# mbjd/binaural-audio-synthesis

Measured on AMD Instinct MI355X. Metric: stereo samples/sec, 256 concurrent moving sources @44.1kHz mixed to one stereo pair (x real-time in x_realtime), higher is better.
Workload: dtype f32

## Files before the change

binaural-audio-synthesis_amd/csrc/bas_fused_split.hip:

```cpp
#include "bas_fused.h"

#ifndef FZ_NT_LOADS
#define FZ_NT_LOADS 1
#endif

#ifndef FS_PSPLIT
#define FS_PSPLIT 1
#endif
#ifndef FS_STAGER_PRIO
#define FS_STAGER_PRIO 3
#endif
#ifndef FS_FILTER_PRIO
#define FS_FILTER_PRIO 0
#endif

#ifdef BAS_STAMPS
__device__ unsigned long long bas_fs_stamps[1024 * 8 * 8];
#define FS_NOW() __builtin_amdgcn_s_memrealtime()
#else
#define FS_NOW() 0ull
#endif

#if FZ_ASM
template <int UNITLEN, int NSUB = 1, int PSPLIT = 0>
__global__ __launch_bounds__(512, 1) void bas_render_fs_kernel(
    FzArgs A, const float *__restrict__ x,
    float *__restrict__ slab,
    const float *__restrict__ packed,
    const unsigned *__restrict__ plans,
    float *__restrict__ y, unsigned int *__restrict__ peak_bits) {
    constexpr int NW = 4;
    constexpr int THREADS = 64 * NW;
    constexpr int TILE = 2048 * NW;
    constexpr int ROWS = TILE / 32 + HD_HALO;
    constexpr int XR = ROWS + 1;
    constexpr int NX = (ROWS * 8 + THREADS - 1) / THREADS;
    constexpr int XFLOATS = 8 * XR * 4;
    constexpr int MAXEV = BAS_FS_MAXEV;
    constexpr int PL4 = 2 * BAS_PLANS_WORDS / 4;
    constexpr int NPV = (MAXEV * PL4 + 63) / 64;
    static_assert(XR == 261, "bas_fir_asm.inc holds the row step for this x-image stride");
    extern __shared__ f32x4 lds4[];
    const int buf4 = (XFLOATS + ((A.nslots * HD_SLOT + 3) & ~3)) / 4;
    f32x4 *pl_base = lds4 + 2 * buf4;
    f32x4 *bnd = pl_base + NW * (MAXEV * PL4);
    volatile unsigned *flags = reinterpret_cast<volatile unsigned *>(bnd + NW * 64);

    const int tid0 = threadIdx.x;
    const int lane0 = tid0 & 63;
    const int wv8 = __builtin_amdgcn_readfirstlane(tid0 >> 6);
    const bool stager = wv8 >= NW;
    const int wv = wv8 & (NW - 1);

    const long unit0 = (long)blockIdx.x * A.units_per_wg;
    long unit1 = unit0 + A.units_per_wg;
    if (unit1 > A.units_total) unit1 = A.units_total;
    const int nseg = (A.Lp + RT_SEG - 1) / RT_SEG;
    const long n_pass = (unit1 - unit0) * nseg;
    if (!A.direct && peak_bits && blockIdx.x == 0 && tid0 == 0) *peak_bits = 0u;
    if (n_pass <= 0) {
        if (A.direct && A.tail_mode) bas_tail<2 * THREADS>(fz_tail(A, y, peak_bits), 0.f);
        return;
    }
    unsigned wmax_bits = 0u;
    if (tid0 < NW) flags[tid0] = 0u;
    __syncthreads();

    const long first_tile = unit0 / A.n_src;
    long tile = first_tile;
    int s = (int)(unit0 - first_tile * A.n_src);
    int sg = 0;
    struct Geo {
        int seg0, Lseg, halo, nrows, c0, mo0;
        long xbase;
    };
    auto make_geo = [&](long t, int g) {
        Geo G;
        G.seg0 = g * RT_SEG;
        G.Lseg = A.Lp - G.seg0 < RT_SEG ? A.Lp - G.seg0 : RT_SEG;
        G.halo = (G.Lseg + 31) >> 5;
        G.xbase = t * TILE - G.seg0 - 32L * G.halo;
        G.nrows = TILE / 32 + G.halo;
        long cf = G.xbase / A.K;
        if (cf * A.K > G.xbase) --cf;
        G.c0 = (int)cf;
        G.mo0 = (int)(G.xbase - cf * A.K);
        return G;
    };
    Geo G = make_geo(tile, sg);
    auto advance = [&]() {
        int n_sg = sg + 1;
        long n_tile = tile;
        if (n_sg == nseg) {
            n_sg = 0;
            if (++s == A.n_src) {
                s = 0;
                ++n_tile;
            }
        }
        if (n_tile != tile || n_sg != sg) G = make_geo(n_tile, n_sg);
        tile = n_tile;
        sg = n_sg;
    };
#ifdef BAS_STAMPS
    unsigned long long st_work = 0, st_wait = 0, st_clk = 0;
    const unsigned long long st_begin = FS_NOW(), st_begin_clk = __builtin_amdgcn_s_memtime();
#endif

    if (!stager) {
        if (FS_FILTER_PRIO) __builtin_amdgcn_s_setprio(FS_FILTER_PRIO);
        static_assert(!PSPLIT || (NSUB == 1 && UNITLEN != 0), "the P split exists for the unit blocks of subchunks >= 32");
        f32x32 accA, accB, accP;
        f32x2 accB16 = f32x2{0.f, 0.f};
        f32x16 accPA, accPB, accPP;
        f32x2 accPB8 = f32x2{0.f, 0.f};
#pragma unroll
        for (int i = 0; i < 32; ++i) accA[i] = accB[i] = accP[i] = 0.f;
#pragma unroll
        for (int i = 0; i < 16; ++i) accPA[i] = accPB[i] = accPP[i] = 0.f;
        float *slab_wg = slab + (long)blockIdx.x * A.parts_per_wg * 2 * TILE;
        auto flush = [&](long t) {
            f32x2 acc[32];
            if constexpr (PSPLIT) {
#pragma unroll
                for (int r = 0; r < 8; ++r) {
                    const f32x2 a = f32x2{accPA[2 * r], accPA[2 * r + 1]}, b0 = f32x2{accPB[2 * r], accPB[2 * r + 1]};
                    const f32x2 b1 = r < 7 ? f32x2{accPB[2 * r + 2], accPB[2 * r + 3]} : accPB8;
                    const f32x2 pp = f32x2{accPP[2 * r], accPP[2 * r + 1]};
                    const f32x2 pe = a + b0, po = (pp - a) - b1;
                    accP[4 * r] = pe.x; accP[4 * r + 1] = pe.y;
                    accP[4 * r + 2] = po.x; accP[4 * r + 3] = po.y;
                }
            }
#pragma unroll
            for (int p = 0; p < 16; ++p) {
                const f32x2 a = f32x2{accA[2 * p], accA[2 * p + 1]}, b0 = f32x2{accB[2 * p], accB[2 * p + 1]};
                const f32x2 b1 = p < 15 ? f32x2{accB[2 * p + 2], accB[2 * p + 3]} : accB16;
                const f32x2 pp = f32x2{accP[2 * p], accP[2 * p + 1]};
                acc[2 * p] = a + b0;
                acc[2 * p + 1] = (pp - a) - b1;
            }
#pragma unroll
            for (int i = 0; i < 32; ++i) accA[i] = accB[i] = accP[i] = 0.f;
            accB16 = f32x2{0.f, 0.f};
            if constexpr (PSPLIT) {
#pragma unroll
                for (int i = 0; i < 16; ++i) accPA[i] = accPB[i] = accPP[i] = 0.f;
                accPB8 = f32x2{0.f, 0.f};
            }
            if (A.direct) {
                const long n0 = t * TILE + 2048 * wv + 32 * lane0;
                const float lmax = fz_store_row_direct(acc, y, A.T_out, n0, A.accumulate);
                if (A.tail_mode) {
                    const unsigned b = fz_wave_max_bits(lmax);
                    wmax_bits = b > wmax_bits ? b : wmax_bits;
                } else if (peak_bits) {
                    bas_wave_peak_max(lmax, peak_bits);
                }
                return;
            }
            float *dst = slab_wg + (t - first_tile) * 2 * TILE + 2048 * wv + 32 * lane0;
            f32x4 *l4 = reinterpret_cast<f32x4 *>(dst);
            f32x4 *r4 = reinterpret_cast<f32x4 *>(dst + TILE);
#pragma unroll
            for (int i = 0; i < 8; ++i) {
                l4[i] = f32x4{acc[4 * i].x, acc[4 * i + 1].x, acc[4 * i + 2].x, acc[4 * i + 3].x};
                r4[i] = f32x4{acc[4 * i].y, acc[4 * i + 1].y, acc[4 * i + 2].y, acc[4 * i + 3].y};
            }
        };
        long open_tile = -1;
        long addr_tile = -1;
        int addr_buf = 0;
        unsigned tapv[5] = {0u, 0u, 0u, 0u, 0u}, xrow4 = 0u;
        float alv[5] = {0.f, 0.f, 0.f, 0.f, 0.f}, blv[5] = {0.f, 0.f, 0.f, 0.f, 0.f};
        const unsigned buf_bytes = 16u * (unsigned)buf4;
        for (long pid = 0; pid < n_pass; ++pid) {
            int tid = tid0;
            asm volatile("" : "+v"(tid));
            const int lane = tid & 63;
#ifdef BAS_STAMPS
            const unsigned long long t0 = FS_NOW();
#endif
            if (tile != open_tile) {
                if (open_tile >= 0) flush(open_tile);
                open_tile = tile;
            }
            auto weight = [&](int m) {
                if (A.s_pow2) return (float)(m & ~(A.S - 1)) * A.invK;
                int q = (int)((float)m * A.invS);
                const int r = m - q * A.S;
                if (r < 0) q -= 1;
                if (r >= A.S) q += 1;
                return (float)(q * A.S) * A.invK;
            };
            if constexpr (UNITLEN != 0) {
                const int cur_buf = (int)(pid & 1);
                const long akey = tile * nseg + sg;
                if (akey == addr_tile && cur_buf != addr_buf) {
                    const unsigned delta = cur_buf ? buf_bytes : 0u - buf_bytes;
#pragma unroll
                    for (int r = 0; r < 5; ++r) tapv[r] += delta;
                    xrow4 += delta;
                    addr_buf = cur_buf;
                }
                if (akey != addr_tile) {
                    addr_tile = akey;
                    addr_buf = cur_buf;
                    const unsigned bufb = (unsigned)reinterpret_cast<uintptr_t>(lds4 + cur_buf * buf4);
                    const int row_out = 64 * wv + lane + G.halo;
                    const int pos = G.mo0 + 32 * row_out;
                    int sl = (int)((float)pos * A.invK);
                    int m_in = pos - sl * A.K;
                    if (m_in < 0) { m_in += A.K; sl -= 1; }
                    if (m_in >= A.K) { m_in -= A.K; sl += 1; }
                    xrow4 = bufb + 16u * (unsigned)(row_out - 4);
                    unsigned tap = bufb + 4u * (unsigned)(XFLOATS + sl * HD_SLOT - 32 * 4);
#pragma unroll
                    for (int r = 0; r < 5; ++r) {
                        alv[r] = weight(m_in);
                        if constexpr (NSUB == 2) blv[r] = weight(m_in + 16);
                        tapv[r] = tap;
                        m_in -= 32;
                        const bool wrap = m_in < 0;
                        m_in += wrap ? A.K : 0;
                        tap += 32u * 16u - (wrap ? 4u * (unsigned)HD_SLOT : 0u);
                    }
                }
            }
#ifdef BAS_STAMPS
            const unsigned long long t1 = FS_NOW();
#endif
            __syncthreads();
#ifdef BAS_STAMPS
            const unsigned long long t2 = FS_NOW();
#endif
            const f32x4 *xs4 = lds4 + (pid & 1) * buf4;
            const float *hd = reinterpret_cast<const float *>(xs4) + XFLOATS;
            const int Lseg = G.Lseg, halo = G.halo;
#ifdef BAS_STAMPS
            const unsigned long long c0 = __builtin_amdgcn_s_memtime();
#endif
            if constexpr (UNITLEN != 0) {
                if constexpr (PSPLIT)
                    ffa_unitp_asm<XR, UNITLEN>(accA, accB, accPA, accPB, accPB8, accPP, accB16, xrow4, tapv, alv);
                else if constexpr (NSUB == 4)
                    ffa_unit4_asm<XR, UNITLEN>(accA, accB, accB16, accP, xrow4, tapv, alv, (float)A.S * A.invK);
                else if constexpr (NSUB == 2)
                    ffa_unit2_asm<XR, UNITLEN>(accA, accB, accB16, accP, xrow4, tapv, alv, blv);
                else
                    ffa_unit_asm<XR, UNITLEN>(accA, accB, accB16, accP, xrow4, tapv, alv);
                (void)hd; (void)Lseg; (void)halo;
            } else {
                const int row_out = 64 * wv + lane + halo;
                const int pos = G.mo0 + 32 * row_out;
                int sl = (int)((float)pos * A.invK);
                int m_in = pos - sl * A.K;
                if (m_in < 0) { m_in += A.K; sl -= 1; }
                if (m_in >= A.K) { m_in -= A.K; sl += 1; }
                const f32x4 *xrow = xs4 + row_out;
#pragma unroll 1
                for (int rp = 0; rp <= halo; ++rp) {
                    float al;
                    if (A.s_pow2) {
                        al = (float)(m_in & ~(A.S - 1)) * A.invK;
                    } else {
                        int q = (int)((float)m_in * A.invS);
                        const int r = m_in - q * A.S;
                        if (r < 0) q -= 1;
                        if (r >= A.S) q += 1;
                        al = (float)(q * A.S) * A.invK;
                    }
                    const int oct_lo = 4 - 4 * rp > 0 ? 4 - 4 * rp : 0;
                    int oct_hi = (Lseg + 32 - 32 * rp) >> 3;
                    oct_hi = oct_hi > 8 ? 8 : oct_hi;
                    const unsigned mk = ((1u << oct_hi) - 1u) & ~((1u << oct_lo) - 1u);
                    ffa_row_step_asm<XR>(accA, accB, accB16, accP, (unsigned)reinterpret_cast<uintptr_t>(xrow),
                                         (unsigned)reinterpret_cast<uintptr_t>(hd + sl * HD_SLOT + (32 * rp - 32) * 4), al, mk);
                    xrow -= 1;
                    m_in -= 32;
                    if (m_in < 0) {
                        m_in += A.K;
                        sl -= 1;
                    }
                }
            }
#ifdef BAS_STAMPS
            st_clk += __builtin_amdgcn_s_memtime() - c0;
            st_work += (t1 - t0) + (FS_NOW() - t2);
            st_wait += t2 - t1;
#endif
            advance();
        }
        flush(open_tile);
    } else {
        __builtin_amdgcn_s_setprio(FS_STAGER_PRIO);
        const __amdgpu_buffer_rsrc_t tab =
            __builtin_amdgcn_make_buffer_rsrc(const_cast<float *>(packed), 0, (int)A.packed_bytes, 0x00020000);
        const unsigned L4 = 4u * (unsigned)A.L;
        const int n_ir = A.nslots + 1, base = n_ir / NW, rem = n_ir - base * NW;
        const int slot_a = rfl(wv * base + (wv < rem ? wv : rem));
        const int slot_b = rfl(slot_a + base + (wv < rem ? 1 : 0));
        const int n_ev = slot_a < slot_b ? slot_b - slot_a : 0;
        const bool need_next = n_ev > 0 && slot_b <= A.nslots;
        f32x4 *plw = pl_base + wv * (MAXEV * PL4);
        const int tid = tid0 - THREADS;
        const int lane = tid & 63;
        const int half = lane >> 5;
        const int tq = 4 * (lane & 31) + (lane < 32 ? 2 : 0);
        const unsigned v16 = 16u * (unsigned)tid, l16 = 16u * (unsigned)lane;
        const bool all_live = A.L == A.Lp;
        for (long pid = 0; pid < n_pass; ++pid) {
#ifdef BAS_STAMPS
            const unsigned long long t0 = FS_NOW();
#endif
#ifndef FS_NO_STAGE
            f32x4 *xs4 = lds4 + (pid & 1) * buf4;
            float *hd = reinterpret_cast<float *>(xs4) + XFLOATS;
            const int seg0 = G.seg0, Lseg = G.Lseg, nrows = G.nrows;
            const long xbase = G.xbase;
            f32x4 pv[NPV], xv[NX];
            {
                const f32x4 *pl_src = reinterpret_cast<const f32x4 *>(plans) + (long)s * (A.n_chunks + 1) * PL4;
                const int c_first = rfl(G.c0 + slot_a);
                if (c_first >= 0 && c_first + n_ev - 1 <= A.n_chunks) {
                    const __amdgpu_buffer_rsrc_t pr = __builtin_amdgcn_make_buffer_rsrc(
                        const_cast<f32x4 *>(pl_src + (long)c_first * PL4), 0, n_ev * PL4 * 16, 0x00020000);
#pragma unroll
                    for (int r = 0; r < NPV; ++r)
                        pv[r] = __builtin_bit_cast(f32x4, __builtin_amdgcn_raw_buffer_load_b128(pr, (int)l16, 1024 * r, FZ_NT_LOADS ? 2 : 0));
                } else {
#pragma unroll
                    for (int r = 0; r < NPV; ++r) {
                        int p = lane + 64 * r;
                        p = p < n_ev * PL4 ? p : 0;
                        const int i = (p * 3641) >> 16;
                        const int c = clampi(c_first + i, 0, A.n_chunks);
#if FZ_NT_LOADS
                        pv[r] = __builtin_nontemporal_load(pl_src + (long)c * PL4 + (p - i * PL4));
#else
                        pv[r] = pl_src[(long)c * PL4 + (p - i * PL4)];
#endif
                    }
                }
            }
            const long lo_l = -xbase, hi_l = A.T_in - xbase;
            const int x_lo = lo_l < -(1 << 30) ? -(1 << 30) : (lo_l > (1 << 30) ? (1 << 30) : (int)lo_l);
            const int x_hi = hi_l < -(1 << 30) ? -(1 << 30) : (hi_l > (1 << 30) ? (1 << 30) : (int)hi_l);
            const bool x_inside = x_lo <= 0 && x_hi >= 4 * NX * THREADS;
            {
                const float *xwin = x + (long)s * A.x_stride + xbase;
                if (x_inside) {
                    const __amdgpu_buffer_rsrc_t xr = __builtin_amdgcn_make_buffer_rsrc(const_cast<float *>(xwin), 0,
                                                                                        16 * NX * THREADS, 0x00020000);
#pragma unroll
                    for (int j = 0; j < NX; ++j)
                        xv[j] = __builtin_bit_cast(f32x4, __builtin_amdgcn_raw_buffer_load_b128(xr, (int)v16, 16 * THREADS * j, FZ_NT_LOADS ? 2 : 0));
                } else {
                    asm volatile("" ::: "memory");
#pragma unroll
                    for (int j = 0; j < NX; ++j) {
                        int i = 4 * (tid + j * THREADS);
                        i = i < x_lo ? x_lo : i;
                        i = i > x_hi - 4 ? x_hi - 4 : i;
#if FZ_NT_LOADS
                        xv[j] = __builtin_nontemporal_load(reinterpret_cast<const f32x4 *>(xwin + i));
#else
                        xv[j] = *reinterpret_cast<const f32x4 *>(xwin + i);
#endif
                    }
                }
            }
            const unsigned pass_id = (unsigned)pid + 1u;
#pragma unroll
            for (int r = 0; r < NPV; ++r)
                if (lane + 64 * r < n_ev * PL4) plw[lane + 64 * r] = pv[r];
            {
                f32x4 *xcol = xs4 + (tid & 7) * XR + (tid >> 3);
                if (!x_inside) {
                    asm volatile("" ::: "memory");
#pragma unroll
                    for (int j = 0; j < NX; ++j) {
                        const int e = 4 * (tid + j * THREADS);
                        if (!(e >= x_lo && e < x_hi)) xv[j] = f32x4{0.f, 0.f, 0.f, 0.f};
                    }
                }
#pragma unroll
                for (int j = 0; j < NX; ++j) {
                    if ((j + 1) * THREADS <= (TILE / 32 + 1) * 8 || tid + j * THREADS < nrows * 8) xcol[32 * j] = xv[j];
                }
            }
            __builtin_amdgcn_wave_barrier();

            {
                const int m = seg0 + 4 * (lane & 31);
                const int m_c = m < A.L ? m : A.L - 1;
                const unsigned m4 = 4u * (unsigned)m_c;
                const f32x4 live = f32x4{m < A.L ? 1.f : 0.f, m + 1 < A.L ? 1.f : 0.f, m + 2 < A.L ? 1.f : 0.f,
                                         m + 3 < A.L ? 1.f : 0.f};
                const f32x4 *pl = plw + half * (BAS_PLANS_WORDS / 4);
                f32x4 *dst = reinterpret_cast<f32x4 *>(hd) + slot_a * (HD_SLOT / 4) + tq;
                FzHalf ha, hb;
                f32x2 pa = f32x2{0.f, 0.f}, pb = pa;
                const f32x4 *pl_last = pl + (n_ev > 0 ? n_ev - 1 : 0) * PL4;
                if (n_ev > 0) fz_issue<0>(tab, pl, m4, L4, ha);
                for (int i = 0; i < n_ev; ++i) {
                    const f32x4 *pl_next = pl + PL4 < pl_last ? pl + PL4 : pl_last;
                    fz_issue<1>(tab, pl, m4, L4, hb);
                    f32x4 h = fz_finish<0>(pl, ha, f32x4{0.f, 0.f, 0.f, 0.f});
                    fz_issue<0>(tab, pl_next, m4, L4, ha);
                    h = fz_finish<1>(pl, hb, h);
                    if (!all_live) h *= live;
                    if (i == 0 && wv > 0) {
                        bnd[wv * 64 + lane] = h;
                        __builtin_amdgcn_fence(__ATOMIC_RELEASE, "workgroup");
                        if (lane == 0 && !fz_inject(A)) flags[wv] = pass_id;
                    }
                    f32x2 ca, cb;
                    fz_pair_ears(h, ca, cb);
                    if (i > 0) {
                        const f32x2 da = ca - pa, db = cb - pb;
                        if (tq < Lseg) {
                            dst[0] = f32x4{pa.x, pa.y, da.x, da.y};
                            dst[1] = f32x4{pb.x, pb.y, db.x, db.y};
                        }
                        dst += HD_SLOT / 4;
                    }
                    pa = ca;
                    pb = cb;
                    pl = pl_next;
                }
                if (need_next) {
                    const bool got = fz_wait_handover(flags + wv + 1, pass_id, A);
                    __builtin_amdgcn_fence(__ATOMIC_ACQUIRE, "workgroup");
                    f32x4 nx = bnd[(wv + 1) * 64 + lane];
                    if (!got) nx = f32x4{__builtin_nanf(""), __builtin_nanf(""), __builtin_nanf(""), __builtin_nanf("")};
                    f32x2 ca, cb;
                    fz_pair_ears(nx, ca, cb);
                    const f32x2 da = ca - pa, db = cb - pb;
                    if (tq < Lseg) {
                        dst[0] = f32x4{pa.x, pa.y, da.x, da.y};
                        dst[1] = f32x4{pb.x, pb.y, db.x, db.y};
                    }
                }
            }
#endif
#ifdef BAS_STAMPS
            asm volatile("s_waitcnt vmcnt(0) lgkmcnt(0)" ::: "memory");
            const unsigned long long t1 = FS_NOW();
#endif
            __syncthreads();
#ifdef BAS_STAMPS
            st_work += t1 - t0;
            st_wait += FS_NOW() - t1;
#endif
            advance();
        }
    }
    if (A.direct && A.tail_mode) bas_tail<2 * THREADS>(fz_tail(A, y, peak_bits), __uint_as_float(wmax_bits));
#ifdef BAS_STAMPS
    if (lane0 == 0 && blockIdx.x < 1024) {
        unsigned long long *d = bas_fs_stamps + (blockIdx.x * 8 + wv8) * 8;
        d[0] = st_work;
        d[1] = st_wait;
        d[2] = st_clk;
        d[3] = __builtin_amdgcn_s_memtime() - st_begin_clk;
        d[6] = FS_NOW() - st_begin;
        d[7] = (unsigned long long)n_pass;
    }
#endif
}

#ifdef BAS_STAMPS
extern "C" int bas_debug_read_fs_stamps(unsigned long long *host, size_t count) {
    return (int)hipMemcpyFromSymbol(host, HIP_SYMBOL(bas_fs_stamps), count * sizeof(unsigned long long));
}
#endif

#endif

int bas_fs_unit_len(int Lp) {
    return FS_UNIT_BLOCK && (Lp == 104 || (Lp > 0 && Lp % 128 == 0)) ? (Lp == 104 ? 104 : 128) : 0;
}

size_t bas_fs_lds_bytes(int nslots) {
    const int rows = 8192 / 32 + HD_HALO;
    return (size_t)(2 * (8 * (rows + 1) * 4 + ((nslots * HD_SLOT + 3) & ~3)) + 4 * BAS_FS_MAXEV * 2 * BAS_PLANS_WORDS + 4 * 64 * 4 + 4) *
           sizeof(float);
}

hipError_t bas_fs_launch(const FzArgs &A, const float *x, float *slab, const float *packed, const unsigned *plans, float *y,
                         unsigned int *peak_bits, int n_wg, size_t lds_bytes, hipStream_t st, hipEvent_t eb, hipEvent_t ee) {
#if FZ_ASM
    typedef void (*fs_fn)(FzArgs, const float *, float *, const float *, const unsigned *, float *, unsigned int *);
    const int ul = bas_fs_unit_len(A.Lp);
#if FS_PSPLIT
    fs_fn fn = ul == 128 ? bas_render_fs_kernel<128, 1, 1> : ul == 104 ? bas_render_fs_kernel<104, 1, 1> : bas_render_fs_kernel<0>;
#else
    fs_fn fn = ul == 128 ? bas_render_fs_kernel<128> : ul == 104 ? bas_render_fs_kernel<104> : bas_render_fs_kernel<0>;
#endif
    if (A.S == 16 || A.S == 8) {
        if (ul == 0) return hipErrorNotSupported;
        fn = A.S == 16 ? (ul == 128 ? bas_render_fs_kernel<128, 2> : bas_render_fs_kernel<104, 2>)
                       : (ul == 128 ? bas_render_fs_kernel<128, 4> : bas_render_fs_kernel<104, 4>);
    }
    hipError_t e = bas_allow_full_lds(reinterpret_cast<const void *>(fn));
    if (e != hipSuccess) return e;
    if (eb) (void)hipEventRecord(eb, st);
    hipLaunchKernelGGL(fn, dim3(n_wg), dim3(512), lds_bytes, st, A, x, slab, packed, plans, y, peak_bits);
    if (ee) (void)hipEventRecord(ee, st);
    return hipSuccess;
#else
    return hipErrorNotSupported;
#endif
}
```

binaural-audio-synthesis_amd/csrc/bas_plan.h:

```cpp
#pragma once
#include "bas_internal.h"

#ifndef BAS_PLANE_DOUBLE
#define BAS_PLANE_DOUBLE 0
#endif
#if BAS_PLANE_DOUBLE
#define BAS_PLANE(L) (2 * (L) + 4)
#else
#define BAS_PLANE(L) ((L) + 4)
#endif

static inline long bas_table_floats(int ndir, int L, int U) {
    if (ndir <= 0 || L <= 0 || U <= 0) return -1;
    const __int128 f = (__int128)2 * ndir * U * BAS_PLANE((__int128)L);
    return f < ((__int128)1 << 31) ? (long)f : -1;
}

#define BAS_PLAN_MIN_U 4

#define BAS_PLANS_WORDS 36
struct EarPlanS {
    unsigned off[16];
    float w[16];
    unsigned o4[4];
};

__device__ __forceinline__ int rfl(int v) { return __builtin_amdgcn_readfirstlane(v); }

typedef float f32x4_a4 __attribute__((ext_vector_type(4), aligned(4)));
typedef unsigned u32x4 __attribute__((ext_vector_type(4)));

struct FzHalf {
    u32x4 v[8];
};

__device__ __forceinline__ unsigned fz_wrap(unsigned m4, unsigned o4, unsigned L4) {
#if BAS_PLANE_DOUBLE
    return m4 + o4;
#endif
    const unsigned idx = m4 + o4;
    const unsigned wr = idx - L4;
    return idx < wr ? idx : wr;
}

template <int HSEL>
__device__ __forceinline__ void fz_issue(__amdgpu_buffer_rsrc_t tab, const f32x4 *__restrict__ pl, unsigned m4,
                                          unsigned L4, FzHalf &H) {
    const u32x4 o4 = __builtin_bit_cast(u32x4, pl[8]);
    const u32x4 pa = __builtin_bit_cast(u32x4, pl[2 * HSEL]), pb = __builtin_bit_cast(u32x4, pl[2 * HSEL + 1]);
    unsigned a[8];
    if (HSEL == 0) {
        const unsigned s0 = fz_wrap(m4, o4.x, L4), s1 = fz_wrap(m4, o4.y, L4);
        a[0] = s0 + pa.x; a[1] = s0 + pa.y; a[2] = s0 + pa.z; a[3] = s0 + pa.w;
        a[4] = s0 + pb.x; a[5] = s1 + pb.y; a[6] = s1 + pb.z; a[7] = s1 + pb.w;
    } else {
        const unsigned s1 = fz_wrap(m4, o4.y, L4), s2 = fz_wrap(m4, o4.z, L4), s3 = fz_wrap(m4, o4.w, L4);
        a[0] = s1 + pa.x; a[1] = s2 + pa.y; a[2] = s2 + pa.z; a[3] = s2 + pa.w;
        a[4] = s2 + pb.x; a[5] = s3 + pb.y; a[6] = s3 + pb.z; a[7] = s3 + pb.w;
    }
#pragma unroll
    for (int j = 0; j < 8; ++j) H.v[j] = __builtin_amdgcn_raw_buffer_load_b128(tab, (int)a[j], 0, 0);
}

template <int HSEL>
__device__ __forceinline__ f32x4 fz_finish(const f32x4 *__restrict__ pl, const FzHalf &H, f32x4 acc) {
    const f32x4 wa = pl[4 + 2 * HSEL], wb = pl[5 + 2 * HSEL];
#pragma unroll
    for (int j = 0; j < 8; ++j) {
        const float w = j < 4 ? wa[j] : wb[j - 4];
        acc = __builtin_elementwise_fma(__builtin_bit_cast(f32x4, H.v[j]), f32x4{w, w, w, w}, acc);
    }
    return acc;
}
```

Before: 710.8 million.

## Rebalance x-window staging across stager waves by IR event load

The stager waves previously each loaded a fixed strided share of the x input window, using block-wide thread indices. Now each wave stages a per-wave range of 64-lane quads. When IR events split unevenly across waves, waves holding fewer IR slots take more x quads, so per-wave work in the staging pass is intended to even out. The change also adds several compile-time ablation switches and a cache-policy knob for table loads, all off by default. The risk is that extra index arithmetic and the branch on the even split could offset the balance gain.

Result: no change. 710.0 million (-0.1%).

```diff
diff --git a/binaural-audio-synthesis_amd/csrc/bas_fused_split.hip b/binaural-audio-synthesis_amd/csrc/bas_fused_split.hip
--- a/binaural-audio-synthesis_amd/csrc/bas_fused_split.hip
+++ b/binaural-audio-synthesis_amd/csrc/bas_fused_split.hip
@@ -14,6 +14,16 @@
 #define FS_FILTER_PRIO 0
 #endif
 
+#ifndef FS_NXW
+#define FS_NXW 13
+#endif
+#ifndef FS_XQ_PER_IR
+#define FS_XQ_PER_IR 8
+#endif
+#if defined(FS_ABL_NO_FOLD) || defined(FS_ABL_NO_LDS_WR)
+#define FS_KEEP(v) asm volatile("" ::"v"(v))
+#endif
+
 #ifdef BAS_STAMPS
 __device__ unsigned long long bas_fs_stamps[1024 * 8 * 8];
 #define FS_NOW() __builtin_amdgcn_s_memrealtime()
@@ -21,7 +31,78 @@
 #define FS_NOW() 0ull
 #endif
 
+#ifdef FS_ABL_NO_TAB
+__device__ __forceinline__ void fs_abl_opaque(FzHalf &H) {
+#pragma unroll
+    for (int j = 0; j < 8; ++j) asm volatile("" : "+v"(H.v[j]));
+}
+#endif
+#ifdef FS_ABL_NO_FOLD
+template <int HSEL>
+__device__ __forceinline__ f32x4 fs_abl_no_fold(const f32x4 *__restrict__ pl, const FzHalf &H, f32x4 acc) {
+    FS_KEEP(pl[4 + 2 * HSEL]);
+    FS_KEEP(pl[5 + 2 * HSEL]);
+#pragma unroll
+    for (int j = 0; j < 8; ++j) FS_KEEP(H.v[j]);
+    return HSEL ? f32x4{1e-3f, 1e-3f, 1e-3f, 1e-3f} : acc;
+}
+#endif
+
 #if FZ_ASM
+template <int XS, int NJ, int NXW, int WINDOW_BYTES>
+__device__ __forceinline__ void fs_x_fetch(f32x4 (&xv)[NXW], const float *xwin, int lane, bool x_inside, int x_lo, int x_hi, int qf,
+                                           int ql, int qn) {
+    if (x_inside) {
+        const __amdgpu_buffer_rsrc_t xr = __builtin_amdgcn_make_buffer_rsrc(const_cast<float *>(xwin), 0,
+                                                                            WINDOW_BYTES, 0x00020000);
+#pragma unroll
+        for (int j = 0; j < NJ; ++j)
+            if (j < qn)
+                xv[j] = __builtin_bit_cast(f32x4, __builtin_amdgcn_raw_buffer_load_b128(xr, 16 * lane, 1024 * (j == 0 ? ql : qf + XS * (j - 1)), FZ_NT_LOADS ? 2 : 0));
+    } else {
+        asm volatile("" ::: "memory");
+#pragma unroll
+        for (int j = 0; j < NJ; ++j) {
+            if (j >= qn) continue;
+            int i = 4 * (64 * (j == 0 ? ql : qf + XS * (j - 1)) + lane);
+            i = i < x_lo ? x_lo : i;
+            i = i > x_hi - 4 ? x_hi - 4 : i;
+#if FZ_NT_LOADS
+            xv[j] = __builtin_nontemporal_load(reinterpret_cast<const f32x4 *>(xwin + i));
+#else
+            xv[j] = *reinterpret_cast<const f32x4 *>(xwin + i);
+#endif
+        }
+    }
+}
+template <int XS, int NJ, int NXW, int XR, int FULL_Q>
+__device__ __forceinline__ void fs_x_store(f32x4 (&xv)[NXW], f32x4 *xs4, int lane, bool x_inside, int x_lo, int x_hi, int nrows, int qf,
+                                           int ql, int qn) {
+    f32x4 *xcol = xs4 + (lane & 7) * XR + (lane >> 3);
+    if (!x_inside) {
+        asm volatile("" ::: "memory");
+#pragma unroll
+        for (int j = 0; j < NJ; ++j) {
+            const int e = 4 * (64 * (j == 0 ? ql : qf + XS * (j - 1)) + lane);
+            if (j < qn && !(e >= x_lo && e < x_hi)) xv[j] = f32x4{0.f, 0.f, 0.f, 0.f};
+        }
+    }
+    f32x4 *xcf = xcol + 8 * qf;
+#pragma unroll
+    for (int j = 0; j < NJ; ++j) {
+        if (j >= qn) continue;
+#ifdef FS_ABL_NO_LDS_WR
+        FS_KEEP(xv[j]);
+#else
+        if (j == 0) {
+            if (ql < FULL_Q || 64 * ql + lane < nrows * 8) xcol[8 * ql] = xv[0];
+        } else {
+            xcf[8 * XS * (j - 1)] = xv[j];
+        }
+#endif
+    }
+}
+
 template <int UNITLEN, int NSUB = 1, int PSPLIT = 0>
 __global__ __launch_bounds__(512, 1) void bas_render_fs_kernel(
     FzArgs A, const float *__restrict__ x,
@@ -35,6 +116,8 @@
     constexpr int ROWS = TILE / 32 + HD_HALO;
     constexpr int XR = ROWS + 1;
     constexpr int NX = (ROWS * 8 + THREADS - 1) / THREADS;
+    constexpr int NQ = (ROWS * 8 + 63) / 64;
+    constexpr int NXW = FS_NXW;
     constexpr int XFLOATS = 8 * XR * 4;
     constexpr int MAXEV = BAS_FS_MAXEV;
     constexpr int PL4 = 2 * BAS_PLANS_WORDS / 4;
@@ -303,11 +386,26 @@
         const int n_ev = slot_a < slot_b ? slot_b - slot_a : 0;
         const bool need_next = n_ev > 0 && slot_b <= A.nslots;
         f32x4 *plw = pl_base + wv * (MAXEV * PL4);
+        int xq0 = wv, xqn = (NQ - wv + NW - 1) / NW;
+        if (rem != 0) {
+            int cl = (NQ + rem * FS_XQ_PER_IR + NW - 1) / NW;
+            cl = cl < NXW ? cl : NXW;
+            const int lt = cl * (NW - rem) < NQ ? cl * (NW - rem) : NQ, ht = NQ - lt;
+            const int ch = (ht + rem - 1) / rem;
+            const int q_a = wv < rem ? wv * ch : ht + (wv - rem) * cl;
+            int q_b = q_a + (wv < rem ? ch : cl);
+            const int q_end = wv < rem ? ht : NQ;
+            q_b = q_b < q_end ? q_b : q_end;
+            xq0 = q_a;
+            xqn = q_b > q_a ? q_b - q_a : 0;
+        }
+        const bool x_even = rem == 0;
+        const int xq_pack = rfl(xq0 | (xq0 + (x_even ? NW : 1) * (xqn > 0 ? xqn - 1 : 0)) << 8 | xqn << 16);
         const int tid = tid0 - THREADS;
         const int lane = tid & 63;
         const int half = lane >> 5;
         const int tq = 4 * (lane & 31) + (lane < 32 ? 2 : 0);
-        const unsigned v16 = 16u * (unsigned)tid, l16 = 16u * (unsigned)lane;
+        const unsigned l16 = 16u * (unsigned)lane;
         const bool all_live = A.L == A.Lp;
         for (long pid = 0; pid < n_pass; ++pid) {
 #ifdef BAS_STAMPS
@@ -318,7 +416,7 @@
             float *hd = reinterpret_cast<float *>(xs4) + XFLOATS;
             const int seg0 = G.seg0, Lseg = G.Lseg, nrows = G.nrows;
             const long xbase = G.xbase;
-            f32x4 pv[NPV], xv[NX];
+            f32x4 pv[NPV], xv[NXW];
             {
                 const f32x4 *pl_src = reinterpret_cast<const f32x4 *>(plans) + (long)s * (A.n_chunks + 1) * PL4;
                 const int c_first = rfl(G.c0 + slot_a);
@@ -347,48 +445,29 @@
             const int x_lo = lo_l < -(1 << 30) ? -(1 << 30) : (lo_l > (1 << 30) ? (1 << 30) : (int)lo_l);
             const int x_hi = hi_l < -(1 << 30) ? -(1 << 30) : (hi_l > (1 << 30) ? (1 << 30) : (int)hi_l);
             const bool x_inside = x_lo <= 0 && x_hi >= 4 * NX * THREADS;
+            int xpk = xq_pack;
+            asm volatile("" : "+v"(xpk));
+            xpk = rfl(xpk);
+            const int qf = xpk & 255, ql = (xpk >> 8) & 255, qn = xpk >> 16;
+#ifndef FS_ABL_NO_X
             {
                 const float *xwin = x + (long)s * A.x_stride + xbase;
-                if (x_inside) {
-                    const __amdgpu_buffer_rsrc_t xr = __builtin_amdgcn_make_buffer_rsrc(const_cast<float *>(xwin), 0,
-                                                                                        16 * NX * THREADS, 0x00020000);
-#pragma unroll
-                    for (int j = 0; j < NX; ++j)
-                        xv[j] = __builtin_bit_cast(f32x4, __builtin_amdgcn_raw_buffer_load_b128(xr, (int)v16, 16 * THREADS * j, FZ_NT_LOADS ? 2 : 0));
-                } else {
-                    asm volatile("" ::: "memory");
-#pragma unroll
-                    for (int j = 0; j < NX; ++j) {
-                        int i = 4 * (tid + j * THREADS);
-                        i = i < x_lo ? x_lo : i;
-                        i = i > x_hi - 4 ? x_hi - 4 : i;
-#if FZ_NT_LOADS
-                        xv[j] = __builtin_nontemporal_load(reinterpret_cast<const f32x4 *>(xwin + i));
-#else
-                        xv[j] = *reinterpret_cast<const f32x4 *>(xwin + i);
-#endif
-                    }
-                }
-            }
+                if (x_even)
+                    fs_x_fetch<NW, (NQ + NW - 1) / NW, NXW, 16 * NX * THREADS>(xv, xwin, lane, x_inside, x_lo, x_hi, qf, ql, qn);
+                else
+                    fs_x_fetch<1, NXW, NXW, 16 * NX * THREADS>(xv, xwin, lane, x_inside, x_lo, x_hi, qf, ql, qn);
+            }
+#endif
             const unsigned pass_id = (unsigned)pid + 1u;
 #pragma unroll
             for (int r = 0; r < NPV; ++r)
                 if (lane + 64 * r < n_ev * PL4) plw[lane + 64 * r] = pv[r];
-            {
-                f32x4 *xcol = xs4 + (tid & 7) * XR + (tid >> 3);
-                if (!x_inside) {
-                    asm volatile("" ::: "memory");
-#pragma unroll
-                    for (int j = 0; j < NX; ++j) {
-                        const int e = 4 * (tid + j * THREADS);
-                        if (!(e >= x_lo && e < x_hi)) xv[j] = f32x4{0.f, 0.f, 0.f, 0.f};
-                    }
-                }
-#pragma unroll
-                for (int j = 0; j < NX; ++j) {
-                    if ((j + 1) * THREADS <= (TILE / 32 + 1) * 8 || tid + j * THREADS < nrows * 8) xcol[32 * j] = xv[j];
-                }
-            }
+#ifndef FS_ABL_NO_X
+            if (x_even)
+                fs_x_store<NW, (NQ + NW - 1) / NW, NXW, XR, (TILE / 32 + 1) * 8 / 64>(xv, xs4, lane, x_inside, x_lo, x_hi, nrows, qf, ql, qn);
+            else
+                fs_x_store<1, NXW, NXW, XR, (TILE / 32 + 1) * 8 / 64>(xv, xs4, lane, x_inside, x_lo, x_hi, nrows, qf, ql, qn);
+#endif
             __builtin_amdgcn_wave_barrier();
 
             {
@@ -402,13 +481,47 @@
                 FzHalf ha, hb;
                 f32x2 pa = f32x2{0.f, 0.f}, pb = pa;
                 const f32x4 *pl_last = pl + (n_ev > 0 ? n_ev - 1 : 0) * PL4;
-                if (n_ev > 0) fz_issue<0>(tab, pl, m4, L4, ha);
+#ifdef FS_ABL_NO_TAB
+#pragma unroll
+                for (int j = 0; j < 8; ++j) ha.v[j] = hb.v[j] = u32x4{0u, 0u, 0u, 0u};
+#endif
+#ifdef FS_ABL_PLAN_REGS
+                f32x4 preg[9];
+#pragma unroll
+                for (int k = 0; k < 9; ++k) {
+                    preg[k] = pl[k];
+                    asm volatile("" : "+v"(preg[k]));
+                }
+#define FS_PL(p) preg
+#else
+#define FS_PL(p) p
+#endif
+#ifdef FS_ABL_NO_TAB
+#define FS_ISSUE(H, p, h) fs_abl_opaque(h)
+#else
+#define FS_ISSUE(H, p, h) fz_issue<H>(tab, FS_PL(p), m4, L4, h)
+#endif
+#ifdef FS_ABL_NO_FOLD
+#define FS_FINISH(H, p, h, acc) fs_abl_no_fold<H>(p, h, acc)
+#else
+#define FS_FINISH(H, p, h, acc) fz_finish<H>(FS_PL(p), h, acc)
+#endif
+#ifdef FS_ABL_FOLD_PRIO
+#define FS_PRIO(p) __builtin_amdgcn_s_setprio(p)
+#else
+#define FS_PRIO(p) (void)0
+#endif
+                if (n_ev > 0) FS_ISSUE(0, pl, ha);
                 for (int i = 0; i < n_ev; ++i) {
                     const f32x4 *pl_next = pl + PL4 < pl_last ? pl + PL4 : pl_last;
-                    fz_issue<1>(tab, pl, m4, L4, hb);
-                    f32x4 h = fz_finish<0>(pl, ha, f32x4{0.f, 0.f, 0.f, 0.f});
-                    fz_issue<0>(tab, pl_next, m4, L4, ha);
-                    h = fz_finish<1>(pl, hb, h);
+                    FS_ISSUE(1, pl, hb);
+                    FS_PRIO(FS_FILTER_PRIO);
+                    f32x4 h = FS_FINISH(0, pl, ha, (f32x4{0.f, 0.f, 0.f, 0.f}));
+                    FS_PRIO(FS_STAGER_PRIO);
+                    FS_ISSUE(0, pl_next, ha);
+                    FS_PRIO(FS_FILTER_PRIO);
+                    h = FS_FINISH(1, pl, hb, h);
+                    FS_PRIO(FS_STAGER_PRIO);
                     if (!all_live) h *= live;
                     if (i == 0 && wv > 0) {
                         bnd[wv * 64 + lane] = h;
@@ -419,10 +532,15 @@
                     fz_pair_ears(h, ca, cb);
                     if (i > 0) {
                         const f32x2 da = ca - pa, db = cb - pb;
+#ifdef FS_ABL_NO_LDS_WR
+                        FS_KEEP(da);
+                        FS_KEEP(db);
+#else
                         if (tq < Lseg) {
                             dst[0] = f32x4{pa.x, pa.y, da.x, da.y};
                             dst[1] = f32x4{pb.x, pb.y, db.x, db.y};
                         }
+#endif
                         dst += HD_SLOT / 4;
                     }
                     pa = ca;
@@ -437,10 +555,15 @@
                     f32x2 ca, cb;
                     fz_pair_ears(nx, ca, cb);
                     const f32x2 da = ca - pa, db = cb - pb;
+#ifdef FS_ABL_NO_LDS_WR
+                    FS_KEEP(da);
+                    FS_KEEP(db);
+#else
                     if (tq < Lseg) {
                         dst[0] = f32x4{pa.x, pa.y, da.x, da.y};
                         dst[1] = f32x4{pb.x, pb.y, db.x, db.y};
                     }
+#endif
                 }
             }
 #endif
diff --git a/binaural-audio-synthesis_amd/csrc/bas_plan.h b/binaural-audio-synthesis_amd/csrc/bas_plan.h
--- a/binaural-audio-synthesis_amd/csrc/bas_plan.h
+++ b/binaural-audio-synthesis_amd/csrc/bas_plan.h
@@ -30,6 +30,9 @@
 typedef float f32x4_a4 __attribute__((ext_vector_type(4), aligned(4)));
 typedef unsigned u32x4 __attribute__((ext_vector_type(4)));
 
+#ifndef FZ_TAB_AUX
+#define FZ_TAB_AUX 0
+#endif
 struct FzHalf {
     u32x4 v[8];
 };
@@ -59,7 +62,7 @@
         a[4] = s2 + pb.x; a[5] = s3 + pb.y; a[6] = s3 + pb.z; a[7] = s3 + pb.w;
     }
 #pragma unroll
-    for (int j = 0; j < 8; ++j) H.v[j] = __builtin_amdgcn_raw_buffer_load_b128(tab, (int)a[j], 0, 0);
+    for (int j = 0; j < 8; ++j) H.v[j] = __builtin_amdgcn_raw_buffer_load_b128(tab, (int)a[j], 0, FZ_TAB_AUX);
 }
 
 template <int HSEL>
```
